# iwa-shi/CRDR

Measured on AMD Instinct MI355X. Metric: stage-3 training img/s at 256x256, higher is better.
Workload: dtype fp32; 1 GPU; config/crdr_stage_3.yaml -b 16: full GAN step (G + 5x CLIC21GVAE D + LPIPS-Alex, random-init weights), rate index cycled 0..4; global_batch=16, crop=256, parallelism=dp1

## Files before the change

### crdr_amd/csrc/wino4_wgrad.hip

```cpp
#include <algorithm>
#include <atomic>
#include <type_traits>

#include "common.hpp"
#include "wgrad_args.hpp"
#include "wino4_xform.hpp"

namespace crdr {

namespace {

typedef __attribute__((address_space(3))) void* lds_ptr_t;
constexpr unsigned kOob = 0x80000000u;
constexpr int kPC = 64, kQC = 32;
constexpr int kPFloats = 4 * 16 * kPC, kQFloats = 6 * 18 * kQC;
constexpr int kUsed = kPFloats + kQFloats;
constexpr int kPieces = kUsed / 4;
constexpr int kPasses = (kPieces + 255) / 256;
constexpr int kStage = ((kPieces + 63) / 64) * 64 * 4;

__device__ __forceinline__ void v4_pk(const f32x2v p0, const f32x2v p1, const f32x2v p2, const f32x2v p3, f32x2v (&o)[6], const W4Consts& kc) {
  f32x2v ea, da, eb, db;
  asm volatile(
      "v_pk_fma_f32 %4, %10, %14, %8 op_sel_hi:[1,0,1]\n"
      "v_pk_fma_f32 %5, %11, %14, %9 op_sel_hi:[1,0,1]\n"
      "v_pk_fma_f32 %6, %10, %14, %8 op_sel:[0,1,0] op_sel_hi:[1,1,1]\n"
      "v_pk_fma_f32 %7, %11, %14, %9 op_sel:[0,1,0] op_sel_hi:[1,1,1]\n"
      "v_pk_fma_f32 %0, %5, %12, %4 op_sel_hi:[1,0,1]\n"
      "v_pk_fma_f32 %1, %5, %13, %4 op_sel_hi:[1,0,1]\n"
      "v_pk_fma_f32 %2, %7, %12, %6 op_sel:[0,1,0] op_sel_hi:[1,1,1]\n"
      "v_pk_fma_f32 %3, %7, %13, %6 op_sel:[0,1,0] op_sel_hi:[1,1,1]"
      : "=&v"(o[1]), "=&v"(o[2]), "=&v"(o[3]), "=&v"(o[4]), "=&v"(ea), "=&v"(da), "=&v"(eb), "=&v"(db)
      : "v"(p0), "v"(p1), "v"(p2), "v"(p3), "s"(kc.k2), "s"(kc.k3), "s"(kc.k5));
  o[0] = p0;
  o[5] = p3;
}

__device__ __forceinline__ float acc_read(float v) {
  float o;
  asm volatile("v_accvgpr_read_b32 %0, %1" : "=v"(o) : "a"(v));
  return o;
}

__global__ __launch_bounds__(256) void wino4_wgrad_kernel(const WgradArgs p_, const WgradGroup grp) {
  extern __shared__ __attribute__((aligned(16))) float smem[];
  const int tid = threadIdx.x, lane = tid & 63, wave = __builtin_amdgcn_readfirstlane(tid >> 6);
  const int iw = wave & 1, jw = wave >> 1;
  WgradArgs p = p_;
  const int gidx = blockIdx.z;
  if (p.ngroup > 1) { p.p = grp.p[gidx]; p.q = grp.q[gidx]; }
  const int nij = ((p.PC + kPC - 1) / kPC) * p.jtiles;
  const int sub = blockIdx.x / nij, bxy = blockIdx.x - sub * nij;
  const int sa = sub >> 1, sb = sub & 1;
  int qs = 1, oy = -p.pad, ox = -p.pad, tap0 = 0, tstep = 1, na = 3, nb = 3;
  if (p.kw == 5 && p.stride == 1) { oy += 3 * sa; ox += 3 * sb; tap0 = (3 * sa) * 5 + 3 * sb; na = sa ? 2 : 3; nb = sb ? 2 : 3; }
  if (p.kw == 5 && p.stride == 2) { qs = 2; oy = sa - 2; ox = sb - 2; tap0 = sa * 5 + sb; tstep = 2; na = sa ? 2 : 3; nb = sb ? 2 : 3; }
  const int it = bxy / p.jtiles, jt = bxy - it * p.jtiles;
  const int i0 = it * kPC, j0 = jt * kQC;
  const int split = blockIdx.y;
  const int TR = (p.PH + 3) >> 2, SC = (p.PW + 15) >> 4;
  const long long S = (long long)p.N * TR * SC;
  const int s0 = (int)(S * split / p.nsplit), s1 = (int)(S * (split + 1) / p.nsplit);
  const __amdgpu_buffer_rsrc_t rp = __builtin_amdgcn_make_buffer_rsrc(const_cast<float*>(p.p), 0, p.p_bytes, 0x00020000);
  const __amdgpu_buffer_rsrc_t rq = __builtin_amdgcn_make_buffer_rsrc(const_cast<float*>(p.q), 0, p.q_bytes, 0x00020000);

  int s_row[kPasses], s_col[kPasses];
  static_assert(kPFloats / 4 == 4 * 256, "staging passes 0..3 are P pieces, 4..7 Q pieces");
  unsigned s_off[kPasses];
#pragma unroll
  for (int j = 0; j < kPasses; ++j) {
    const int Sx = tid + 256 * j;
    const bool isp = Sx < kPFloats / 4;
    const int px = isp ? Sx >> 4 : (Sx - kPFloats / 4) >> 3;
    const int ch = isp ? (Sx & 15) * 4 : ((Sx - kPFloats / 4) & 7) * 4;
    s_row[j] = isp ? px >> 4 : px / 18;
    s_col[j] = isp ? px & 15 : px - (px / 18) * 18;
    if (isp) s_off[j] = i0 + ch < p.PC ? (unsigned)(((s_row[j] * p.PW + s_col[j]) * p.ldp + i0 + ch) * 4) : kOob;
    else s_off[j] = j0 + ch < p.QC ? (unsigned)(((qs * s_row[j] * p.QW + qs * s_col[j]) * p.ldq + j0 + ch) * 4) : kOob;
    if (Sx >= kPieces) s_off[j] = kOob;
  }
  const int last_pass = wave < 2 ? kPasses - 1 : kPasses - 2;
  if (wave >= 2) { s_off[kPasses - 1] = s_off[kPasses - 2]; s_row[kPasses - 1] = s_row[kPasses - 2]; s_col[kPasses - 1] = s_col[kPasses - 2]; }
  int f_n, f_tr, f_sc;
  {
    const int n = s0 / (TR * SC), rem = s0 - n * (TR * SC);
    f_n = n; f_tr = rem / SC; f_sc = rem - f_tr * SC;
  }
  int fn = 0, ftr = 0, fsc = 0;
  unsigned f_dp = 0, f_dq = 0;
  bool f_inner = true, f_live = true;
  auto fetch_begin = [&](bool live) __attribute__((always_inline)) {
    fn = f_n; ftr = f_tr; fsc = f_sc;
    if (++f_sc == SC) { f_sc = 0; if (++f_tr == TR) { f_tr = 0; ++f_n; } }
    f_live = live;
    f_dp = (unsigned)((((fn * p.PH + 4 * ftr) * p.PW + 16 * fsc) * p.ldp) * 4);
    f_inner = 4 * ftr + 4 <= p.PH && 16 * fsc + 16 <= p.PW && qs * 4 * ftr + oy >= 0 && qs * (4 * ftr + 5) + oy < p.QH &&
              qs * 16 * fsc + ox >= 0 && qs * (16 * fsc + 17) + ox < p.QW;
    f_dq = (unsigned)((((fn * p.QH + qs * 4 * ftr + oy) * p.QW + qs * 16 * fsc + ox) * p.ldq) * 4);
  };
  unsigned off8[kPasses];
  unsigned f_sq = 0;
  auto fetch_offsets = [&]() __attribute__((always_inline)) {
#pragma unroll
    for (int j = 0; j < kPasses; ++j) off8[j] = s_off[j];
    f_sq = f_dq;
    if (!f_inner) {
      f_sq = 0;
#pragma unroll
      for (int j = 0; j < kPasses; ++j) {
        if (j < 4) {
          const int a = 4 * ftr + s_row[j], b = 16 * fsc + s_col[j];
          if (!(a < p.PH && b < p.PW)) off8[j] = kOob;
        } else {
          const int a = qs * (4 * ftr + s_row[j]) + oy, b = qs * (16 * fsc + s_col[j]) + ox;
          off8[j] = ((unsigned)a < (unsigned)p.QH && (unsigned)b < (unsigned)p.QW && s_off[j] != kOob) ? s_off[j] + f_dq : kOob;
        }
      }
    }
  };
  auto fetch_piece = [&](int buf, int j) __attribute__((always_inline)) {
    const int jd = j == kPasses - 1 ? last_pass : j;
    float* st = smem + buf * kStage;
    const __amdgpu_buffer_rsrc_t rl = f_live ? (j < 4 ? rp : rq) : __builtin_amdgcn_make_buffer_rsrc(nullptr, 0, 0, 0x00020000);
    __builtin_amdgcn_raw_ptr_buffer_load_lds(rl, (lds_ptr_t)(st + (jd * 256 + wave * 64) * 4), 16, (int)off8[j], (int)(j < 4 ? f_dp : f_sq), 0, 0);
  };

  f32x4 acc[64], accv[8];
#pragma unroll
  for (int j = 0; j < 64; ++j) acc[j] = f32x4{0.f, 0.f, 0.f, 0.f};
#pragma unroll
  for (int j = 0; j < 8; ++j) accv[j] = f32x4{0.f, 0.f, 0.f, 0.f};

  const int m = lane & 15, kg = lane >> 4;
  const int pb = (4 * kg) * kPC + 32 * iw + m, qb = kPFloats + (4 * kg) * kQC + 16 * jw + m;
  const W4Consts kc = w4_consts();
  f32x2v PR[4][4];
  f32x2v QR[3][6];
  f32x2v Ap[6][6];
  f32x2v Vq[6][3];
  auto raw_read = [&](const float* st, int r) __attribute__((always_inline)) {
    if (r < 16) {
      const int u = r >> 2, v = r & 3;
      PR[u][v] = f32x2v{st[pb + (u * 16 + v) * kPC], st[pb + (u * 16 + v) * kPC + 16]};
    } else {
      const int c = (r - 16) / 6, u = (r - 16) - 6 * c;
      QR[c][u] = f32x2v{st[qb + (u * 18 + 2 * c) * kQC], st[qb + (u * 18 + 2 * c + 1) * kQC]};
    }
  };
  auto transforms = [&]() __attribute__((always_inline)) {
    {
      f32x2v t[6][4];
#pragma unroll
      for (int v = 0; v < 4; ++v) {
        f32x2v o[6];
        v4_pk(PR[0][v], PR[1][v], PR[2][v], PR[3][v], o, kc);
#pragma unroll
        for (int x = 0; x < 6; ++x) t[x][v] = o[x];
      }
      __builtin_amdgcn_sched_barrier(0);
#pragma unroll
      for (int x = 0; x < 6; ++x) v4_pk(t[x][0], t[x][1], t[x][2], t[x][3], Ap[x], kc);
      __builtin_amdgcn_sched_barrier(0);
    }
    {
      f32x2v T[6][3];
#pragma unroll
      for (int c = 0; c < 3; ++c) {
        f32x2v t6[6];
        bt6_cols(QR[c], t6, kc);
#pragma unroll
        for (int x = 0; x < 6; ++x) T[x][c] = t6[x];
      }
      __builtin_amdgcn_sched_barrier(0);
#pragma unroll
      for (int x = 0; x < 6; ++x) bt6_row(T[x][0], T[x][1], T[x][2], Vq[x], kc);
      __builtin_amdgcn_sched_barrier(0);
    }
  };
  auto mfma_slot = [&](int s) __attribute__((always_inline)) {
    const int pos = s >> 1, ib = s & 1, x = pos / 6, y = pos - 6 * x;
    const float av = ib ? Ap[x][y].y : Ap[x][y].x;
    if (s < 64) acc[s] = __builtin_amdgcn_mfma_f32_16x16x4f32(av, v_elem(Vq[x], y), acc[s], 0, 0, 0);
    else asm volatile("v_mfma_f32_16x16x4_f32 %0, %1, %2, %0" : "+v"(accv[s - 64]) : "v"(av), "v"(v_elem(Vq[x], y)));
  };
  if (s0 < s1) {
    fetch_begin(true);
    fetch_offsets();
#pragma unroll
    for (int j = 0; j < kPasses; ++j) fetch_piece(0, j);
    __builtin_amdgcn_s_waitcnt(0x0070);
    __syncthreads();
    fetch_begin(s0 + 1 < s1);
    fetch_offsets();
#pragma unroll
    for (int j = 0; j < kPasses; ++j) fetch_piece(1, j);
#pragma unroll
    for (int r = 0; r < 34; ++r) raw_read(smem, r);
  }
  for (int s = s0; s < s1; ++s) {
    const int buf = (s - s0) & 1;
    const float* stn = smem + (buf ^ 1) * kStage;
    fetch_begin(s + 2 < s1);
    fetch_offsets();
    __builtin_amdgcn_sched_barrier(0);
    transforms();
#pragma unroll
    for (int t = 0; t < 36; ++t) {
      mfma_slot(t);
      __builtin_amdgcn_sched_barrier(0);
    }
    __builtin_amdgcn_s_waitcnt(0x0070);
    __builtin_amdgcn_s_barrier();
    __builtin_amdgcn_sched_barrier(0);
#pragma unroll
    for (int t = 36; t < 72; ++t) {
      mfma_slot(t);
      const int q = t - 36;
      if (q < kPasses) fetch_piece(buf, q);
      else {
        const int r0 = q - kPasses < 6 ? 2 * (q - kPasses) : (q - kPasses) + 6;
        raw_read(stn, r0);
        if (q - kPasses < 6) raw_read(stn, r0 + 1);
      }
      __builtin_amdgcn_sched_barrier(0);
    }
  }

  float* slab = p.ws + (size_t)gidx * p.slab_elems + (size_t)split * p.T * p.PC * p.QC;
  const int jc = j0 + 16 * jw + m;
  const double D[6] = {1.0 / kWN0, 1.0 / kWNa, 1.0 / kWNa, 1.0 / kWNb, 1.0 / kWNb, 1.0};
#pragma unroll
  for (int ib = 0; ib < 2; ++ib)
#pragma unroll
    for (int r = 0; r < 4; ++r) {
      float sv[3][6];
#pragma unroll
      for (int nu = 0; nu < 6; ++nu) {
        float u[6];
#pragma unroll
        for (int xi = 0; xi < 6; ++xi) {
          const int blk = 2 * (xi * 6 + nu) + ib;
          const float raw = blk < 64 ? acc_read(acc[blk < 64 ? blk : 0][r]) : accv[blk >= 64 ? blk - 64 : 0][r];
          u[xi] = raw * (float)(D[xi] * D[nu]);
        }
        const float pp = u[1] + u[2], qq = u[1] - u[2], uu = u[3] + u[4], ww = u[3] - u[4];
        sv[0][nu] = u[0] + pp + uu;
        sv[1][nu] = __builtin_fmaf(kWb, ww, kWa * qq);
        sv[2][nu] = __builtin_fmaf(kWb2, uu, kWa2 * pp) + u[5];
      }
      const int i = i0 + 32 * iw + 16 * ib + 4 * kg + r;
#pragma unroll
      for (int a = 0; a < 3; ++a) {
        const float pp = sv[a][1] + sv[a][2], qq = sv[a][1] - sv[a][2], uu = sv[a][3] + sv[a][4], ww = sv[a][3] - sv[a][4];
        const float g0 = sv[a][0] + pp + uu, g1 = __builtin_fmaf(kWb, ww, kWa * qq), g2 = __builtin_fmaf(kWb2, uu, kWa2 * pp) + sv[a][5];
        if (i < p.PC && jc < p.QC && a < na) {
          const int t0 = tap0 + tstep * (a * p.kw);
          slab[((size_t)t0 * p.PC + i) * p.QC + jc] = g0;
          slab[((size_t)(t0 + tstep) * p.PC + i) * p.QC + jc] = g1;
          if (nb > 2) slab[((size_t)(t0 + 2 * tstep) * p.PC + i) * p.QC + jc] = g2;
        }
      }
      __builtin_amdgcn_sched_barrier(0);
    }
}

}

void wino4_wgrad_launch(const WgradArgs& a, const WgradGroup& grp, dim3 grid, hipStream_t s) {
  static std::atomic<bool> attr_done{false};
  if (!attr_done.load(std::memory_order_acquire)) {
    (void)hipFuncSetAttribute(reinterpret_cast<const void*>(wino4_wgrad_kernel), hipFuncAttributeMaxDynamicSharedMemorySize, 160 * 1024);
    attr_done.store(true, std::memory_order_release);
  }
  hipLaunchKernelGGL(wino4_wgrad_kernel, grid, dim3(256), (size_t)2 * kStage * sizeof(float), s, a, grp);
}

}
```

Baseline: 220.7 img/s.

## Split Winograd wgrad tile across two wave halves with triple-buffered LDS staging

```diff
diff --git a/crdr_amd/csrc/wino4_wgrad.hip b/crdr_amd/csrc/wino4_wgrad.hip
--- a/crdr_amd/csrc/wino4_wgrad.hip
+++ b/crdr_amd/csrc/wino4_wgrad.hip
@@ -13,12 +13,45 @@
 typedef __attribute__((address_space(3))) void* lds_ptr_t;
 constexpr unsigned kOob = 0x80000000u;
 constexpr int kPC = 64, kQC = 32;
-constexpr int kPFloats = 4 * 16 * kPC, kQFloats = 6 * 18 * kQC;
-constexpr int kUsed = kPFloats + kQFloats;
-constexpr int kPieces = kUsed / 4;
-constexpr int kPasses = (kPieces + 255) / 256;
-constexpr int kStage = ((kPieces + 63) / 64) * 64 * 4;
-
+constexpr int kPGroup = 272, kPFloats = 16 * kPGroup, kQBlocks = 14, kQPix = 6 * 18;
+constexpr int kStage = kPFloats + kQBlocks * 256;
+constexpr int kStages = 3;
+constexpr int kBlocks = 16 + kQBlocks, kPasses = 4;
+constexpr int kXRegion = 9 * 32 * 16 + 16;
+constexpr int kLdsFloats = 8 * kXRegion > kStages * kStage ? 8 * kXRegion : kStages * kStage;
+
+#ifndef W4W_STAGGER
+#define W4W_STAGGER 1
+#endif
+#ifndef W4W_PRIO
+#define W4W_PRIO 1
+#endif
+
+template <int H>
+__device__ __forceinline__ void v4_half(const f32x2v p0, const f32x2v p1, const f32x2v p2, const f32x2v p3, f32x2v (&o)[3], const W4Consts& kc) {
+  f32x2v e, d;
+  if (H == 0) {
+    asm volatile(
+        "v_pk_fma_f32 %2, %6, %10, %4 op_sel_hi:[1,0,1]\n"
+        "v_pk_fma_f32 %3, %7, %10, %5 op_sel_hi:[1,0,1]\n"
+        "s_nop 0\n"
+        "v_pk_fma_f32 %0, %3, %8, %2 op_sel_hi:[1,0,1]\n"
+        "v_pk_fma_f32 %1, %3, %9, %2 op_sel_hi:[1,0,1]"
+        : "=&v"(o[1]), "=&v"(o[2]), "=&v"(e), "=&v"(d)
+        : "v"(p0), "v"(p1), "v"(p2), "v"(p3), "s"(kc.k2), "s"(kc.k3), "s"(kc.k5));
+    o[0] = p0;
+  } else {
+    asm volatile(
+        "v_pk_fma_f32 %2, %6, %10, %4 op_sel:[0,1,0] op_sel_hi:[1,1,1]\n"
+        "v_pk_fma_f32 %3, %7, %10, %5 op_sel:[0,1,0] op_sel_hi:[1,1,1]\n"
+        "s_nop 0\n"
+        "v_pk_fma_f32 %0, %3, %8, %2 op_sel:[0,1,0] op_sel_hi:[1,1,1]\n"
+        "v_pk_fma_f32 %1, %3, %9, %2 op_sel:[0,1,0] op_sel_hi:[1,1,1]"
+        : "=&v"(o[0]), "=&v"(o[1]), "=&v"(e), "=&v"(d)
+        : "v"(p0), "v"(p1), "v"(p2), "v"(p3), "s"(kc.k2), "s"(kc.k3), "s"(kc.k5));
+    o[2] = p3;
+  }
+}
 __device__ __forceinline__ void v4_pk(const f32x2v p0, const f32x2v p1, const f32x2v p2, const f32x2v p3, f32x2v (&o)[6], const W4Consts& kc) {
   f32x2v ea, da, eb, db;
   asm volatile(
@@ -35,17 +68,78 @@
   o[0] = p0;
   o[5] = p3;
 }
-
-__device__ __forceinline__ float acc_read(float v) {
-  float o;
-  asm volatile("v_accvgpr_read_b32 %0, %1" : "=v"(o) : "a"(v));
-  return o;
-}
-
-__global__ __launch_bounds__(256) void wino4_wgrad_kernel(const WgradArgs p_, const WgradGroup grp) {
+template <int H>
+__device__ __forceinline__ void bt6_cols_half(const f32x2v da, const f32x2v d1, const f32x2v d2, const f32x2v d3, const f32x2v d4, f32x2v (&T)[3],
+                                              const W4Consts& kc) {
+  f32x2v e, o, x;
+  if (H == 0) {
+    asm volatile(
+        "v_pk_fma_f32 %3, %8, %11, %10 op_sel_hi:[1,0,1]\n"
+        "v_pk_fma_f32 %4, %7, %11, %9 op_sel_hi:[1,0,1]\n"
+        "v_pk_fma_f32 %5, %8, %14, %10 op_sel:[0,1,0] op_sel_hi:[1,1,1]\n"
+        "v_pk_fma_f32 %1, %4, %12, %3 op_sel_hi:[1,0,1]\n"
+        "v_pk_fma_f32 %2, %4, %13, %3 op_sel_hi:[1,0,1]\n"
+        "v_pk_fma_f32 %0, %6, %14, %5 op_sel_hi:[1,0,1]"
+        : "=&v"(T[0]), "=&v"(T[1]), "=&v"(T[2]), "=&v"(e), "=&v"(o), "=&v"(x)
+        : "v"(da), "v"(d1), "v"(d2), "v"(d3), "v"(d4), "s"(kc.k1), "s"(kc.k2), "s"(kc.k3), "s"(kc.k4));
+  } else {
+    asm volatile(
+        "v_pk_fma_f32 %3, %8, %11, %10 op_sel:[0,1,0] op_sel_hi:[1,1,1]\n"
+        "v_pk_fma_f32 %4, %7, %11, %9 op_sel:[0,1,0] op_sel_hi:[1,1,1]\n"
+        "v_pk_fma_f32 %5, %9, %14, %6 op_sel:[0,1,0] op_sel_hi:[1,1,1]\n"
+        "v_pk_fma_f32 %0, %4, %12, %3 op_sel:[0,1,0] op_sel_hi:[1,1,1]\n"
+        "v_pk_fma_f32 %1, %4, %13, %3 op_sel:[0,1,0] op_sel_hi:[1,1,1]\n"
+        "v_pk_fma_f32 %2, %7, %14, %5 op_sel_hi:[1,0,1]"
+        : "=&v"(T[0]), "=&v"(T[1]), "=&v"(T[2]), "=&v"(e), "=&v"(o), "=&v"(x)
+        : "v"(da), "v"(d1), "v"(d2), "v"(d3), "v"(d4), "s"(kc.k1), "s"(kc.k2), "s"(kc.k3), "s"(kc.k4));
+  }
+}
+
+typedef f32x4 acc_t;
+
+template <int H>
+__device__ __forceinline__ void half_output_transform(const acc_t (&acc)[32], const acc_t (&accv)[4], float* xr) {
+  const double D[6] = {1.0 / kWN0, 1.0 / kWNa, 1.0 / kWNa, 1.0 / kWNb, 1.0 / kWNb, 1.0};
+#pragma unroll
+  for (int ib = 0; ib < 2; ++ib)
+#pragma unroll
+    for (int r = 0; r < 4; ++r) {
+      float sv[3][6];
+#pragma unroll
+      for (int nu = 0; nu < 6; ++nu) {
+        float u[3];
+#pragma unroll
+        for (int lx = 0; lx < 3; ++lx) {
+          const int blk = 2 * (lx * 6 + nu) + ib;
+          u[lx] = (blk < 32 ? acc[blk < 32 ? blk : 0][r] : accv[blk >= 32 ? blk - 32 : 0][r]) * (float)(D[3 * H + lx] * D[nu]);
+        }
+        if (H == 0) {
+          const float pp = u[1] + u[2], qq = u[1] - u[2];
+          sv[0][nu] = u[0] + pp;
+          sv[1][nu] = kWa * qq;
+          sv[2][nu] = kWa2 * pp;
+        } else {
+          const float uu = u[0] + u[1], ww = u[0] - u[1];
+          sv[0][nu] = uu;
+          sv[1][nu] = kWb * ww;
+          sv[2][nu] = __builtin_fmaf(kWb2, uu, u[2]);
+        }
+      }
+#pragma unroll
+      for (int a = 0; a < 3; ++a) {
+        const float pp = sv[a][1] + sv[a][2], qq = sv[a][1] - sv[a][2], uu = sv[a][3] + sv[a][4], ww = sv[a][3] - sv[a][4];
+        xr[(3 * a + 0) * 512 + (4 * ib + r) * 64] = sv[a][0] + pp + uu;
+        xr[(3 * a + 1) * 512 + (4 * ib + r) * 64] = __builtin_fmaf(kWb, ww, kWa * qq);
+        xr[(3 * a + 2) * 512 + (4 * ib + r) * 64] = __builtin_fmaf(kWb2, uu, kWa2 * pp) + sv[a][5];
+      }
+      __builtin_amdgcn_sched_barrier(0);
+    }
+}
+
+__global__ __launch_bounds__(512) void wino4_wgrad_kernel(const WgradArgs p_, const WgradGroup grp) {
   extern __shared__ __attribute__((aligned(16))) float smem[];
   const int tid = threadIdx.x, lane = tid & 63, wave = __builtin_amdgcn_readfirstlane(tid >> 6);
-  const int iw = wave & 1, jw = wave >> 1;
+  const int iw = wave & 1, jw = (wave >> 1) & 1, h = wave >> 2;
   WgradArgs p = p_;
   const int gidx = blockIdx.z;
   if (p.ngroup > 1) { p.p = grp.p[gidx]; p.q = grp.q[gidx]; }
@@ -61,26 +155,29 @@
   const int TR = (p.PH + 3) >> 2, SC = (p.PW + 15) >> 4;
   const long long S = (long long)p.N * TR * SC;
   const int s0 = (int)(S * split / p.nsplit), s1 = (int)(S * (split + 1) / p.nsplit);
-  const __amdgpu_buffer_rsrc_t rp = __builtin_amdgcn_make_buffer_rsrc(const_cast<float*>(p.p), 0, p.p_bytes, 0x00020000);
-  const __amdgpu_buffer_rsrc_t rq = __builtin_amdgcn_make_buffer_rsrc(const_cast<float*>(p.q), 0, p.q_bytes, 0x00020000);
-
-  int s_row[kPasses], s_col[kPasses];
-  static_assert(kPFloats / 4 == 4 * 256, "staging passes 0..3 are P pieces, 4..7 Q pieces");
+
+  int s_rc[kPasses];
   unsigned s_off[kPasses];
+  int s_dst[kPasses];
 #pragma unroll
   for (int j = 0; j < kPasses; ++j) {
-    const int Sx = tid + 256 * j;
-    const bool isp = Sx < kPFloats / 4;
-    const int px = isp ? Sx >> 4 : (Sx - kPFloats / 4) >> 3;
-    const int ch = isp ? (Sx & 15) * 4 : ((Sx - kPFloats / 4) & 7) * 4;
-    s_row[j] = isp ? px >> 4 : px / 18;
-    s_col[j] = isp ? px & 15 : px - (px / 18) * 18;
-    if (isp) s_off[j] = i0 + ch < p.PC ? (unsigned)(((s_row[j] * p.PW + s_col[j]) * p.ldp + i0 + ch) * 4) : kOob;
-    else s_off[j] = j0 + ch < p.QC ? (unsigned)(((qs * s_row[j] * p.QW + qs * s_col[j]) * p.ldq + j0 + ch) * 4) : kOob;
-    if (Sx >= kPieces) s_off[j] = kOob;
-  }
-  const int last_pass = wave < 2 ? kPasses - 1 : kPasses - 2;
-  if (wave >= 2) { s_off[kPasses - 1] = s_off[kPasses - 2]; s_row[kPasses - 1] = s_row[kPasses - 2]; s_col[kPasses - 1] = s_col[kPasses - 2]; }
+    int b = 8 * j + wave;
+    if (b >= kBlocks) b -= 8;
+    if (j < 2) {
+      const int row = b >> 2, col = 4 * (b & 3) + (lane >> 4), ch = (lane & 15) * 4;
+      s_rc[j] = row | col << 8;
+      s_off[j] = i0 + ch < p.PC ? (unsigned)(((row * p.PW + col) * p.ldp + i0 + ch) * 4) : kOob;
+      s_dst[j] = b * kPGroup;
+    } else {
+      const int k = b - 16, sp = lane >> 3;
+      const int px = 8 * k + (((sp >> 1) & 1) | ((sp >> 2) & 1) << 1 | (sp & 1) << 2);
+      const int ch = ((lane & 7) ^ ((k & 1) << 2)) * 4;
+      const int row = px / 18, col = px - row * 18;
+      s_rc[j] = row | col << 8;
+      s_off[j] = (px < kQPix && j0 + ch < p.QC) ? (unsigned)(((qs * row * p.QW + qs * col) * p.ldq + j0 + ch) * 4) : kOob;
+      s_dst[j] = kPFloats + k * 256;
+    }
+  }
   int f_n, f_tr, f_sc;
   {
     const int n = s0 / (TR * SC), rem = s0 - n * (TR * SC);
@@ -88,180 +185,206 @@
   }
   int fn = 0, ftr = 0, fsc = 0;
   unsigned f_dp = 0, f_dq = 0;
-  bool f_inner = true, f_live = true;
+  bool f_inner = true;
+  unsigned f_pb = 0, f_qb = 0;
   auto fetch_begin = [&](bool live) __attribute__((always_inline)) {
     fn = f_n; ftr = f_tr; fsc = f_sc;
     if (++f_sc == SC) { f_sc = 0; if (++f_tr == TR) { f_tr = 0; ++f_n; } }
-    f_live = live;
+    f_pb = live ? p.p_bytes : 0u; f_qb = live ? p.q_bytes : 0u;
     f_dp = (unsigned)((((fn * p.PH + 4 * ftr) * p.PW + 16 * fsc) * p.ldp) * 4);
     f_inner = 4 * ftr + 4 <= p.PH && 16 * fsc + 16 <= p.PW && qs * 4 * ftr + oy >= 0 && qs * (4 * ftr + 5) + oy < p.QH &&
               qs * 16 * fsc + ox >= 0 && qs * (16 * fsc + 17) + ox < p.QW;
     f_dq = (unsigned)((((fn * p.QH + qs * 4 * ftr + oy) * p.QW + qs * 16 * fsc + ox) * p.ldq) * 4);
   };
-  unsigned off8[kPasses];
+  unsigned off4[kPasses];
   unsigned f_sq = 0;
   auto fetch_offsets = [&]() __attribute__((always_inline)) {
 #pragma unroll
-    for (int j = 0; j < kPasses; ++j) off8[j] = s_off[j];
+    for (int j = 0; j < kPasses; ++j) off4[j] = s_off[j];
     f_sq = f_dq;
     if (!f_inner) {
       f_sq = 0;
 #pragma unroll
       for (int j = 0; j < kPasses; ++j) {
-        if (j < 4) {
-          const int a = 4 * ftr + s_row[j], b = 16 * fsc + s_col[j];
-          if (!(a < p.PH && b < p.PW)) off8[j] = kOob;
+        const int row = s_rc[j] & 255, col = s_rc[j] >> 8;
+        if (j < 2) {
+          const int a = 4 * ftr + row, b = 16 * fsc + col;
+          if (!(a < p.PH && b < p.PW)) off4[j] = kOob;
         } else {
-          const int a = qs * (4 * ftr + s_row[j]) + oy, b = qs * (16 * fsc + s_col[j]) + ox;
-          off8[j] = ((unsigned)a < (unsigned)p.QH && (unsigned)b < (unsigned)p.QW && s_off[j] != kOob) ? s_off[j] + f_dq : kOob;
+          const int a = qs * (4 * ftr + row) + oy, b = qs * (16 * fsc + col) + ox;
+          off4[j] = ((unsigned)a < (unsigned)p.QH && (unsigned)b < (unsigned)p.QW && s_off[j] != kOob) ? s_off[j] + f_dq : kOob;
         }
       }
     }
   };
-  auto fetch_piece = [&](int buf, int j) __attribute__((always_inline)) {
-    const int jd = j == kPasses - 1 ? last_pass : j;
-    float* st = smem + buf * kStage;
-    const __amdgpu_buffer_rsrc_t rl = f_live ? (j < 4 ? rp : rq) : __builtin_amdgcn_make_buffer_rsrc(nullptr, 0, 0, 0x00020000);
-    __builtin_amdgcn_raw_ptr_buffer_load_lds(rl, (lds_ptr_t)(st + (jd * 256 + wave * 64) * 4), 16, (int)off8[j], (int)(j < 4 ? f_dp : f_sq), 0, 0);
-  };
-
-  f32x4 acc[64], accv[8];
-#pragma unroll
-  for (int j = 0; j < 64; ++j) acc[j] = f32x4{0.f, 0.f, 0.f, 0.f};
-#pragma unroll
-  for (int j = 0; j < 8; ++j) accv[j] = f32x4{0.f, 0.f, 0.f, 0.f};
+  auto fetch_piece = [&](float* st, int j) __attribute__((always_inline)) {
+    const __amdgpu_buffer_rsrc_t rl = j < 2 ? __builtin_amdgcn_make_buffer_rsrc(const_cast<float*>(p.p), 0, f_pb, 0x00020000)
+                                            : __builtin_amdgcn_make_buffer_rsrc(const_cast<float*>(p.q), 0, f_qb, 0x00020000);
+    __builtin_amdgcn_raw_ptr_buffer_load_lds(rl, (lds_ptr_t)(st + s_dst[j]), 16, (int)off4[j], (int)(j < 2 ? f_dp : f_sq), 0, 0);
+  };
+
+  acc_t acc[32], accv[4];
+#pragma unroll
+  for (int j = 0; j < 32; ++j) acc[j] = acc_t{0.f, 0.f, 0.f, 0.f};
+#pragma unroll
+  for (int j = 0; j < 4; ++j) accv[j] = acc_t{0.f, 0.f, 0.f, 0.f};
 
   const int m = lane & 15, kg = lane >> 4;
-  const int pb = (4 * kg) * kPC + 32 * iw + m, qb = kPFloats + (4 * kg) * kQC + 16 * jw + m;
+  const int pb = kg * kPGroup + 32 * iw + m;
+  int ql[2][2];
+#pragma unroll
+  for (int b2 = 0; b2 < 2; ++b2)
+#pragma unroll
+    for (int bk = 0; bk < 2; ++bk) {
+      const int e = b2 + kg;
+      ql[b2][bk] = kPFloats + (e >> 1) * 256 + (e & 1) * 32 + ((16 * jw + m) ^ (((bk + (e >> 1)) & 1) << 4));
+    }
   const W4Consts kc = w4_consts();
   f32x2v PR[4][4];
-  f32x2v QR[3][6];
-  f32x2v Ap[6][6];
-  f32x2v Vq[6][3];
-  auto raw_read = [&](const float* st, int r) __attribute__((always_inline)) {
-    if (r < 16) {
-      const int u = r >> 2, v = r & 3;
-      PR[u][v] = f32x2v{st[pb + (u * 16 + v) * kPC], st[pb + (u * 16 + v) * kPC + 16]};
-    } else {
-      const int c = (r - 16) / 6, u = (r - 16) - 6 * c;
-      QR[c][u] = f32x2v{st[qb + (u * 18 + 2 * c) * kQC], st[qb + (u * 18 + 2 * c + 1) * kQC]};
-    }
-  };
-  auto transforms = [&]() __attribute__((always_inline)) {
+  f32x2v QR[3][5];
+  f32x2v Ap[3][6];
+  f32x2v Vq[3][3];
+#pragma unroll
+  for (int x = 0; x < 3; ++x) {
+#pragma unroll
+    for (int y = 0; y < 6; ++y) Ap[x][y] = f32x2v{0.f, 0.f};
+#pragma unroll
+    for (int y = 0; y < 3; ++y) Vq[x][y] = f32x2v{0.f, 0.f};
+  }
+  auto raw_reads = [&](const float* st, auto hc) __attribute__((always_inline)) {
+    constexpr int H = decltype(hc)::value;
+#pragma unroll
+    for (int u = 0; u < 4; ++u)
+#pragma unroll
+      for (int v = 0; v < 4; ++v) {
+        const float* a = st + pb + u * 4 * kPGroup + v * 64;
+        PR[u][v] = f32x2v{a[0], a[16]};
+      }
+#pragma unroll
+    for (int c = 0; c < 3; ++c)
+#pragma unroll
+      for (int uu = 0; uu < 5; ++uu) {
+        const int B = 18 * (uu + H) + 2 * c;
+        const float* a = st + ql[(B >> 2) & 1][(B >> 3) & 1] + (B >> 3) * 256 + ((B >> 1) & 1) * 128;
+        QR[c][uu] = f32x2v{a[0], a[64]};
+      }
+  };
+  auto transforms = [&](auto hc) __attribute__((always_inline)) {
+    constexpr int H = decltype(hc)::value;
     {
-      f32x2v t[6][4];
+      f32x2v T[3][3];
+#pragma unroll
+      for (int c = 0; c < 3; ++c) {
+        f32x2v t3[3];
+        bt6_cols_half<H>(H ? QR[c][4] : QR[c][0], QR[c][1 - H], QR[c][2 - H], QR[c][3 - H], QR[c][4 - H], t3, kc);
+#pragma unroll
+        for (int x = 0; x < 3; ++x) T[x][c] = t3[x];
+      }
+      __builtin_amdgcn_sched_barrier(0);
+#pragma unroll
+      for (int x = 0; x < 3; ++x) bt6_row(T[x][0], T[x][1], T[x][2], Vq[x], kc);
+      __builtin_amdgcn_sched_barrier(0);
+    }
+    {
+      f32x2v t[3][4];
 #pragma unroll
       for (int v = 0; v < 4; ++v) {
-        f32x2v o[6];
-        v4_pk(PR[0][v], PR[1][v], PR[2][v], PR[3][v], o, kc);
-#pragma unroll
-        for (int x = 0; x < 6; ++x) t[x][v] = o[x];
-      }
-      __builtin_amdgcn_sched_barrier(0);
-#pragma unroll
-      for (int x = 0; x < 6; ++x) v4_pk(t[x][0], t[x][1], t[x][2], t[x][3], Ap[x], kc);
-      __builtin_amdgcn_sched_barrier(0);
-    }
-    {
-      f32x2v T[6][3];
-#pragma unroll
-      for (int c = 0; c < 3; ++c) {
-        f32x2v t6[6];
-        bt6_cols(QR[c], t6, kc);
-#pragma unroll
-        for (int x = 0; x < 6; ++x) T[x][c] = t6[x];
-      }
-      __builtin_amdgcn_sched_barrier(0);
-#pragma unroll
-      for (int x = 0; x < 6; ++x) bt6_row(T[x][0], T[x][1], T[x][2], Vq[x], kc);
-      __builtin_amdgcn_sched_barrier(0);
-    }
-  };
-  auto mfma_slot = [&](int s) __attribute__((always_inline)) {
-    const int pos = s >> 1, ib = s & 1, x = pos / 6, y = pos - 6 * x;
-    const float av = ib ? Ap[x][y].y : Ap[x][y].x;
-    if (s < 64) acc[s] = __builtin_amdgcn_mfma_f32_16x16x4f32(av, v_elem(Vq[x], y), acc[s], 0, 0, 0);
-    else asm volatile("v_mfma_f32_16x16x4_f32 %0, %1, %2, %0" : "+v"(accv[s - 64]) : "v"(av), "v"(v_elem(Vq[x], y)));
-  };
+        f32x2v o[3];
+        v4_half<H>(PR[0][v], PR[1][v], PR[2][v], PR[3][v], o, kc);
+#pragma unroll
+        for (int x = 0; x < 3; ++x) t[x][v] = o[x];
+      }
+      __builtin_amdgcn_sched_barrier(0);
+#pragma unroll
+      for (int x = 0; x < 3; ++x) v4_pk(t[x][0], t[x][1], t[x][2], t[x][3], Ap[x], kc);
+      __builtin_amdgcn_sched_barrier(0);
+    }
+  };
+  auto read_and_transform = [&](const float* st, auto hc) __attribute__((always_inline)) {
+    raw_reads(st, hc);
+    __builtin_amdgcn_s_waitcnt(0xc07f);
+    __builtin_amdgcn_sched_barrier(0);
+    transforms(hc);
+  };
+  auto mfmas = [&](float* dst) __attribute__((always_inline)) {
+#pragma unroll
+    for (int t = 0; t < 36; ++t) {
+      const int pos = t >> 1, ib = t & 1, x = pos / 6, y = pos - 6 * x;
+      const float av = ib ? Ap[x][y].y : Ap[x][y].x;
+      if (t < 32) asm volatile("v_mfma_f32_16x16x4_f32 %0, %1, %2, %0" : "+a"(acc[t < 32 ? t : 0]) : "v"(av), "v"(v_elem(Vq[x], y)));
+      else asm volatile("v_mfma_f32_16x16x4_f32 %0, %1, %2, %0" : "+v"(accv[t >= 32 ? t - 32 : 0]) : "v"(av), "v"(v_elem(Vq[x], y)));
+      if (dst != nullptr && t < kPasses) fetch_piece(dst, t);
+      __builtin_amdgcn_sched_barrier(0);
+    }
+  };
+
+  float *st0 = smem, *st1 = smem + kStage, *st2 = smem + 2 * kStage;
   if (s0 < s1) {
     fetch_begin(true);
     fetch_offsets();
 #pragma unroll
-    for (int j = 0; j < kPasses; ++j) fetch_piece(0, j);
-    __builtin_amdgcn_s_waitcnt(0x0070);
-    __syncthreads();
+    for (int j = 0; j < kPasses; ++j) fetch_piece(st0, j);
     fetch_begin(s0 + 1 < s1);
     fetch_offsets();
 #pragma unroll
-    for (int j = 0; j < kPasses; ++j) fetch_piece(1, j);
-#pragma unroll
-    for (int r = 0; r < 34; ++r) raw_read(smem, r);
-  }
-  for (int s = s0; s < s1; ++s) {
-    const int buf = (s - s0) & 1;
-    const float* stn = smem + (buf ^ 1) * kStage;
-    fetch_begin(s + 2 < s1);
-    fetch_offsets();
-    __builtin_amdgcn_sched_barrier(0);
-    transforms();
-#pragma unroll
-    for (int t = 0; t < 36; ++t) {
-      mfma_slot(t);
-      __builtin_amdgcn_sched_barrier(0);
-    }
+    for (int j = 0; j < kPasses; ++j) fetch_piece(st1, j);
+  }
+#if W4W_PRIO
+  if (h) __builtin_amdgcn_s_setprio(1);
+#endif
+  auto half_main = [&](auto hc) __attribute__((always_inline)) {
+    constexpr int H = decltype(hc)::value;
+    for (int s = s0; s < s1; ++s) {
+      fetch_begin(s + 2 < s1);
+      fetch_offsets();
+      __builtin_amdgcn_sched_barrier(0);
+      __builtin_amdgcn_s_waitcnt(0x0f74);
+      __builtin_amdgcn_s_barrier();
+      __builtin_amdgcn_sched_barrier(0);
+      if (H == 0 || !W4W_STAGGER) read_and_transform(st0, hc);
+      mfmas(st2);
+      if (H != 0 && W4W_STAGGER) read_and_transform(st0, hc);
+      __builtin_amdgcn_sched_barrier(0);
+      float* t = st0; st0 = st1; st1 = st2; st2 = t;
+    }
+    if (H != 0 && W4W_STAGGER) mfmas(nullptr);
+    if (H != 0 && W4W_PRIO) __builtin_amdgcn_s_setprio(0);
     __builtin_amdgcn_s_waitcnt(0x0070);
-    __builtin_amdgcn_s_barrier();
-    __builtin_amdgcn_sched_barrier(0);
-#pragma unroll
-    for (int t = 36; t < 72; ++t) {
-      mfma_slot(t);
-      const int q = t - 36;
-      if (q < kPasses) fetch_piece(buf, q);
-      else {
-        const int r0 = q - kPasses < 6 ? 2 * (q - kPasses) : (q - kPasses) + 6;
-        raw_read(stn, r0);
-        if (q - kPasses < 6) raw_read(stn, r0 + 1);
-      }
-      __builtin_amdgcn_sched_barrier(0);
-    }
-  }
-
+    asm volatile("s_nop 15\n s_nop 15" ::: "memory");
+    __syncthreads();
+    half_output_transform<H>(acc, accv, smem + (iw + 2 * jw + 4 * H) * kXRegion + lane);
+  };
+  if (h == 0) half_main(std::integral_constant<int, 0>{});
+  else half_main(std::integral_constant<int, 1>{});
+  __syncthreads();
   float* slab = p.ws + (size_t)gidx * p.slab_elems + (size_t)split * p.T * p.PC * p.QC;
-  const int jc = j0 + 16 * jw + m;
-  const double D[6] = {1.0 / kWN0, 1.0 / kWNa, 1.0 / kWNa, 1.0 / kWNb, 1.0 / kWNb, 1.0};
-#pragma unroll
-  for (int ib = 0; ib < 2; ++ib)
-#pragma unroll
-    for (int r = 0; r < 4; ++r) {
-      float sv[3][6];
-#pragma unroll
-      for (int nu = 0; nu < 6; ++nu) {
-        float u[6];
-#pragma unroll
-        for (int xi = 0; xi < 6; ++xi) {
-          const int blk = 2 * (xi * 6 + nu) + ib;
-          const float raw = blk < 64 ? acc_read(acc[blk < 64 ? blk : 0][r]) : accv[blk >= 64 ? blk - 64 : 0][r];
-          u[xi] = raw * (float)(D[xi] * D[nu]);
+  {
+    int tix = wave * 64 + (int)__builtin_amdgcn_mbcnt_hi(~0u, __builtin_amdgcn_mbcnt_lo(~0u, 0u));
+    asm volatile("" : "+v"(tix));
+    const int jq8 = tix & 7, irow = tix >> 3;
+    const int iw3 = irow >> 5, ilp = irow & 31, jw3 = jq8 >> 2, jq = jq8 & 3;
+    const int i = i0 + 32 * iw3 + 16 * (ilp >> 4) + 4 * (ilp & 3) + ((ilp >> 2) & 3);
+    const int jc = j0 + 16 * jw3 + 4 * jq;
+    const float* xs = smem + (iw3 + 2 * jw3) * kXRegion + ilp * 16 + 4 * jq;
+    const bool vec = (p.QC & 3) == 0 && (reinterpret_cast<size_t>(slab) & 15) == 0;
+    if (i < p.PC && jc < p.QC) {
+#pragma unroll
+      for (int a = 0; a < 3; ++a)
+#pragma unroll
+        for (int b = 0; b < 3; ++b) {
+          if (a < na && b < nb) {
+            const f32x4 v = *reinterpret_cast<const f32x4*>(xs + (3 * a + b) * 512) + *reinterpret_cast<const f32x4*>(xs + 4 * kXRegion + (3 * a + b) * 512);
+            float* o = slab + ((size_t)(tap0 + tstep * (a * p.kw + b)) * p.PC + i) * p.QC + jc;
+            if (vec) *reinterpret_cast<f32x4*>(o) = v;
+            else {
+#pragma unroll
+              for (int jj = 0; jj < 4; ++jj)
+                if (jc + jj < p.QC) o[jj] = v[jj];
+            }
+          }
         }
-        const float pp = u[1] + u[2], qq = u[1] - u[2], uu = u[3] + u[4], ww = u[3] - u[4];
-        sv[0][nu] = u[0] + pp + uu;
-        sv[1][nu] = __builtin_fmaf(kWb, ww, kWa * qq);
-        sv[2][nu] = __builtin_fmaf(kWb2, uu, kWa2 * pp) + u[5];
-      }
-      const int i = i0 + 32 * iw + 16 * ib + 4 * kg + r;
-#pragma unroll
-      for (int a = 0; a < 3; ++a) {
-        const float pp = sv[a][1] + sv[a][2], qq = sv[a][1] - sv[a][2], uu = sv[a][3] + sv[a][4], ww = sv[a][3] - sv[a][4];
-        const float g0 = sv[a][0] + pp + uu, g1 = __builtin_fmaf(kWb, ww, kWa * qq), g2 = __builtin_fmaf(kWb2, uu, kWa2 * pp) + sv[a][5];
-        if (i < p.PC && jc < p.QC && a < na) {
-          const int t0 = tap0 + tstep * (a * p.kw);
-          slab[((size_t)t0 * p.PC + i) * p.QC + jc] = g0;
-          slab[((size_t)(t0 + tstep) * p.PC + i) * p.QC + jc] = g1;
-          if (nb > 2) slab[((size_t)(t0 + 2 * tstep) * p.PC + i) * p.QC + jc] = g2;
-        }
-      }
-      __builtin_amdgcn_sched_barrier(0);
-    }
+    }
+  }
 }
 
 }
@@ -272,7 +395,7 @@
     (void)hipFuncSetAttribute(reinterpret_cast<const void*>(wino4_wgrad_kernel), hipFuncAttributeMaxDynamicSharedMemorySize, 160 * 1024);
     attr_done.store(true, std::memory_order_release);
   }
-  hipLaunchKernelGGL(wino4_wgrad_kernel, grid, dim3(256), (size_t)2 * kStage * sizeof(float), s, a, grp);
-}
-
-}
+  hipLaunchKernelGGL(wino4_wgrad_kernel, grid, dim3(512), (size_t)kLdsFloats * sizeof(float), s, a, grp);
+}
+
+}
```

After: 218.3 img/s (median of 2 runs). 0.989x the previous value.
